# aharley/pips

Measured on AMD Instinct MI355X. Metric: particle-updates/sec (B*S*N*iters/s) at S=8 N=256 368x496, higher is better.
Workload: dtype f32; 1 GPU; BASELINE configs[1]: B=1/GPU S=8 368x496 N=256 I=6 fp32 stride 8, encoder included, inputs resident in HBM; clips_per_gpu=1, parallelism=clip-sharded x1, collective=none

## Files before the change

### include/pips_hip.h

```cpp
#ifndef PIPS_HIP_H
#define PIPS_HIP_H

#include <stddef.h>
#include <stdint.h>

#ifdef __cplusplus
extern "C" {
#endif

#define PIPS_OK            0
#define PIPS_E_ARG        -1
#define PIPS_E_WORKSPACE  -2
#define PIPS_E_LAUNCH     -3

#define PIPS_S        8
#define PIPS_C        128
#define PIPS_LEVELS   4
#define PIPS_RADIUS   3
#define PIPS_NCORR    196
#define PIPS_KIN      519
#define PIPS_KIN_PAD  544
#define PIPS_DMIX     512
#define PIPS_DEPTH    12
#define PIPS_NOUT     1040
// ... 128 lines not shown
                     float* C, int ldc, int M, int N, int K, int epi,
                     const float* R, int ldr, void* stream);
int    pips_conv_nhwc_f32(const float* in, int F, int H, int W, int Cin,
                          const float* wgt, const float* bias, int Cout, int ksize, int cstride, int pad,
                          float* out, float* stats, int* tiles_m_host, void* stream);

#define PIPS_EPI_BIAS      0
#define PIPS_EPI_GELU      1
#define PIPS_EPI_RESIDUAL  2
#define PIPS_EPI_RES_BF16  0x1000
int    pips_gemm_bf16(const void* A, int a_bf16, int lda, const void* W, const float* bias, void* C, int out_bf16, int ldc,
                      int M, int N, int K, int epi, const float* R, int ldr, void* stream);
int    pips_gemm_bf16_route(int M, int N, int K, int epi, int a_bf16, int out_bf16);

int    pips_gemm_f32_route(int M, int N, int K, int epi);
int    pips_device_cus(void);

int    pips_conv_nhwc_bf16(const float* in, int F, int H, int W, int Cin,
                           const void* wgt_bf16, const float* bias, int Cout, int ksize, int cstride, int pad,
                           float* out, float* stats, int* tiles_m_host, void* stream);

int    pips_conv_nhwc_bf16_maps(const void* in_bf16, const float* in_norm, int F, int H, int W, int Cin,
                                const void* wgt_bf16, const float* bias, int Cout, int ksize, int cstride, int pad,
                                void* out, int out_is_bf16, float* stats, int stats_parts_cap, int* tiles_m_host,
                                void* stream);

int    pips_split_bf16x3(const float* src, size_t n, void* dst3, void* stream);
int    pips_gemm_f32x3(const float* A, int lda, const void* W3, const float* bias,
                       float* C, int ldc, int M, int N, int K, int epi,
                       const float* R, int ldr, void* stream);
// ... 26 lines not shown
```

### pips_amd/_lib.py

```python
from __future__ import annotations

import ctypes as C
import os
import threading

HERE = os.path.dirname(os.path.abspath(__file__))
LIB_PATH = os.path.join(HERE, "libpips_hip.so")

c_void_p, c_int, c_size_t, c_float = C.c_void_p, C.c_int, C.c_size_t, C.c_float
fp = c_void_p

SIGNATURES = {
    "pips_last_error": (C.c_char_p, []),
    "pips_abi_version": (c_int, []),
    "pips_weight_arena_bytes": (c_size_t, []),
    "pips_repack_weights": (c_int, [C.POINTER(c_void_p), c_int, c_void_p, c_void_p]),
    "pips_repack_weights_ex": (c_int, [C.POINTER(c_void_p), c_int, c_void_p, c_int, c_void_p]),
    "pips_workspace_bytes": (c_size_t, [c_int] * 6),
    "pips_forward": (c_int, [c_void_p, fp, fp, fp, fp, fp, c_int, c_int, c_int, c_int, c_int, c_int, c_int, c_int,
                             c_void_p, c_size_t, fp, fp, fp, c_void_p]),
    "pips_forward_ce": (c_int, [c_void_p, fp, fp, fp, fp, fp, c_int, c_int, c_int, c_int, c_int, c_int, c_int, c_int,
                                c_void_p, c_size_t, fp, fp, fp, fp, fp, c_void_p, c_size_t, c_void_p]),
    "pips_track_ce": (c_int, [c_void_p, fp, c_int, c_int, c_int, c_int, fp, fp, fp, c_void_p, fp, c_int, c_int, c_int,
                              c_int, c_void_p, c_size_t, fp, fp, fp, fp, fp, c_void_p, c_size_t, c_void_p]),
# ... 45 lines not shown
    "pips_mixer_fwd": (c_int, [c_void_p, fp, c_int, fp, c_void_p, c_size_t, c_void_p]),
    "pips_mixer_fwd_bf16": (c_int, [c_void_p, fp, c_int, fp, c_void_p, c_size_t, c_void_p]),
    "pips_mixer_fwd_x3": (c_int, [c_void_p, fp, c_int, fp, c_void_p, c_size_t, c_void_p]),
    "pips_mixer_fwd_timed": (c_int, [c_void_p, fp, c_int, fp, c_void_p, c_size_t, c_void_p, C.POINTER(c_float)]),
    "pips_mixer_fwd_timed_ex": (c_int, [c_void_p, fp, c_int, c_int, fp, c_void_p, c_size_t, c_void_p,
                                        C.POINTER(c_float)]),
    "pips_mixer_gemm_train": (c_int, [c_void_p, c_int, c_int, c_void_p, c_size_t, c_void_p, c_int, C.POINTER(c_float)]),
    "pips_state_update": (c_int, [c_void_p, fp, fp, fp, fp, c_int, c_int, c_float, fp, fp, c_void_p]),
    "pips_gemm_f32": (c_int, [fp, c_int, fp, fp, fp, c_int, c_int, c_int, c_int, c_int, fp, c_int, c_void_p]),
    "pips_conv_nhwc_f32": (c_int, [fp, c_int, c_int, c_int, c_int, fp, fp, c_int, c_int, c_int, c_int, fp, fp,
                                   C.POINTER(c_int), c_void_p]),
    "pips_gemm_bf16": (c_int, [c_void_p, c_int, c_int, c_void_p, fp, c_void_p, c_int, c_int, c_int, c_int, c_int, c_int, fp, c_int,
                       c_void_p]),
    "pips_gemm_bf16_route": (c_int, [c_int] * 6),
    "pips_gemm_f32_route": (c_int, [c_int] * 4),
    "pips_device_cus": (c_int, []),
    "pips_conv_nhwc_bf16": (c_int, [fp, c_int, c_int, c_int, c_int, c_void_p, fp, c_int, c_int, c_int, c_int, fp, fp,
                                    C.POINTER(c_int), c_void_p]),
    "pips_conv_nhwc_bf16_maps": (c_int, [c_void_p, fp, c_int, c_int, c_int, c_int, c_void_p, fp, c_int, c_int, c_int, c_int,
                                         c_void_p, c_int, fp, c_int, C.POINTER(c_int), c_void_p]),
    "pips_split_bf16x3": (c_int, [fp, c_size_t, c_void_p, c_void_p]),
    "pips_gemm_f32x3": (c_int, [fp, c_int, c_void_p, fp, fp, c_int, c_int, c_int, c_int, c_int, fp, c_int, c_void_p]),
    "pips_conv_nhwc_f32x3": (c_int, [fp, c_int, c_int, c_int, c_int, c_void_p, fp, c_int, c_int, c_int, c_int, fp, fp,
                                     C.POINTER(c_int), c_void_p]),
}

_lock = threading.Lock()
_lib = None


# ... 45 lines not shown
```

### pips_amd/csrc/api.hip

```cpp
#include "common.h"

#include <cstdarg>
#include <cstdio>
#include <cstdlib>
#include <cstring>
#include <mutex>

namespace pips {

static thread_local char g_err[512] = "";

void set_error(const char* fmt, ...) {
    va_list ap;
    va_start(ap, fmt);
    vsnprintf(g_err, sizeof(g_err), fmt, ap);
    va_end(ap);
}

#ifdef PIPS_TUNING
int tune_env(const char* name, int dflt) {
    const char* e = getenv(name);
    return e ? atoi(e) : dflt;
}
#endif
// ... 774 lines not shown
    return gemm_h(reinterpret_cast<const float*>(A), a_bf16, lda, reinterpret_cast<const unsigned short*>(W), bias,
                  reinterpret_cast<float*>(C), out_bf16, ldc, M, N, K, epi, R, ldr, (hipStream_t)stream);
}

int pips_gemm_bf16_route(int M, int N, int K, int epi, int a_bf16, int out_bf16) {
    if (M <= 0 || N <= 0 || K <= 0) return 0;
    static const float dummy = 0.f;
    GemmArgs g;
    memset(&g, 0, sizeof(g));
    g.bias = &dummy; g.R = &dummy;
    g.M = M; g.N = N; g.K = K; g.lda = K; g.ldc = N; g.ldr = N; g.epi = epi;
    return gemm_bf16_asm_route(g, a_bf16, out_bf16);
}

int pips_device_cus(void) { return device_cus(); }

int pips_gemm_f32_route(int M, int N, int K, int epi) {
    if (M <= 0 || N <= 0 || K <= 0) return 0;
    static const float dummy = 0.f;
    GemmArgs g;
    memset(&g, 0, sizeof(g));
    g.bias = &dummy; g.R = &dummy;
    g.M = M; g.N = N; g.K = K; g.lda = K; g.ldc = N; g.ldr = N; g.epi = epi;
    return gemm_f32_t4_route(g, nullptr);
}

static int mixer_mode(int flags) {
    if (flags & PIPS_FLAG_SPLIT_BF16) return 2;
    if (flags & PIPS_FLAG_BF16_MIXER) return (flags & PIPS_FLAG_BF16_STREAM) ? 3 : 1;
    return 0;
// ... 441 lines not shown
```

### pips_amd/csrc/common.h

```cpp
#pragma once
#include <hip/hip_runtime.h>
#include <atomic>
#include <stdint.h>
#include <stddef.h>
#include "../../include/pips_hip.h"

namespace pips {

void set_error(const char* fmt, ...);

#define PIPS_CHECK_ARG(cond, ...)                                   \
    do {                                                            \
        if (!(cond)) { ::pips::set_error(__VA_ARGS__); return PIPS_E_ARG; } \
    } while (0)

#define PIPS_CHECK_LAUNCH(what)                                                     \
    do {                                                                            \
        hipError_t e__ = hipGetLastError();                                         \
        if (e__ != hipSuccess) {                                                    \
            ::pips::set_error("%s: %s", what, hipGetErrorString(e__));              \
            return PIPS_E_LAUNCH;                                                   \
        }                                                                           \
    } while (0)

// ... 197 lines not shown
                    typedef __bf16 bf16x4_ __attribute__((ext_vector_type(4)));
                    const f32x4_ t = {lo.x, lo.y, hi.x, hi.y};
                    bf16x4_ ob = __builtin_convertvector(t, bf16x4_);
                    *reinterpret_cast<uint2*>(reinterpret_cast<unsigned short*>(Cv) + o) = *reinterpret_cast<uint2*>(&ob);
                } else {
                    *reinterpret_cast<float4*>(reinterpret_cast<float*>(Cv) + o) = make_float4(lo.x, lo.y, hi.x, hi.y);
                }
            }
    }
}

int launch_gemm(const GemmArgs& a, hipStream_t st);
int gemm_f32_t4_route(const GemmArgs& a, int* tpb);
int launch_gemm_f32_t4(const GemmArgs& a, int route, int tpb, hipStream_t st);
int launch_conv(const GemmArgs& a, int frames, int* tiles_m, hipStream_t st);
int conv_f32_t4_config(const GemmArgs& a, int frames);
int launch_conv_f32_t4(const GemmArgs& a, int cfg, int frames, int* parts_out, hipStream_t st);
int launch_gemm_bf16(const GemmArgs& a, int a_bf16, int out_bf16, hipStream_t st);
int launch_conv_bf16(const GemmArgs& a, int frames, int* tiles_m, hipStream_t st, int in_bf16 = 0, int out_bf16 = 0);
int launch_conv3x3_c64_bf16(const GemmArgs& a, int frames, int* tiles_m, hipStream_t st, int in_bf16 = 0, int out_bf16 = 0);
bool conv3x3_c64_takes(int H, int W, int frames);
bool conv_c96_t4_takes(const GemmArgs& a, int frames, int in_bf16, int out_bf16);
int launch_conv_c96_t4(const GemmArgs& a, int frames, int* parts_out, hipStream_t st);
int gemm_bf16_asm_route(const GemmArgs& a, int a_bf16, int out_bf16);
bool gemm_bf16_t4_takes(const GemmArgs& a, int a_bf16, int out_bf16);
int launch_gemm_bf16_t4(const GemmArgs& a, hipStream_t st);
bool gemm_bf16_t4up_takes(const GemmArgs& a, int a_bf16, int out_bf16, int* tpb);
int launch_gemm_bf16_t4up(const GemmArgs& a, int tpb, hipStream_t st);
int launch_split_bf16x3(const float* src, size_t n, void* dst, hipStream_t st);
int launch_gemm_x3(const GemmArgs& a, hipStream_t st);
// ... 74 lines not shown
```

### pips_amd/csrc/gemm.hip

```cpp
#include "common.h"

#include <cstdlib>

namespace pips {



template <int BM, int BN, int WGM, int WGN, int KS, bool CONV>
__global__ __launch_bounds__(WGM * WGN * KS * 64, (BM * BN >= 128 * 128 && WGM * WGN * KS == 4) ? 2 : 1) void igemm_f32_kernel(GemmArgs p) {
    constexpr int NT = WGM * WGN * KS * 64;
    constexpr int BKB = 32 * KS;
    constexpr int LD = BKB + 4;
    constexpr int TPR = BKB / 4;
    constexpr int WTM = BM / WGM, WTN = BN / WGN;
    constexpr int TM = WTM / 32, TN = WTN / 32;
    constexpr int ROWS_PER_PASS = NT / TPR;
    constexpr int PA = BM / ROWS_PER_PASS, PB = BN / ROWS_PER_PASS;
    constexpr int STAGE = (BM + BN) * LD;
    static_assert(BM % ROWS_PER_PASS == 0 && BN % ROWS_PER_PASS == 0, "tile/loader mismatch");
    static_assert(WTM % 32 == 0 && WTN % 32 == 0, "wave tile must be 32-granular");
    static_assert(KS == 1 || (KS - 1) * BM * BN <= 2 * STAGE, "K-split reduction does not fit the stages");

    extern __shared__ __attribute__((aligned(16))) float smem[];

    const int tid = threadIdx.x;
    const int lane = tid & 63, wave = tid >> 6;
    const int ks = wave / (WGM * WGN);
    const int wmn = wave - ks * (WGM * WGN);
    const int wm = wmn / WGN, wn = wmn % WGN;
    const int l31 = lane & 31, half = lane >> 5;
    const Tile3 tile_ = xcd_tile_order(p.swz != 0);
    const int bx = tile_.x, by = tile_.y;
    const int m0 = bx * BM, n0 = by * BN;
    const int frame = tile_.z;
#ifdef PIPS_GEMM_TRACE
    unsigned long long* tr_ = p.trace + 8 * (size_t)(blockIdx.x + gridDim.x * (blockIdx.y + gridDim.y * blockIdx.z));
// ... 9 lines not shown
#define PIPS_T(slot)
#endif
    PIPS_T(0)

    const float* __restrict__ Abase = p.A;
    float* __restrict__ Cbase = p.C;
    if (CONV) {
        Abase += (size_t)frame * p.H * p.Win * p.Cin;
        Cbase += (size_t)frame * p.M * p.ldc;
    }

    const int lrow = tid / TPR, cg = tid % TPR;
    static_assert(PA <= 4 && PB <= 6, "extend the pass macros");
#define PIPS_PASSES_A(X) X(0) X(1) X(2) X(3)
#define PIPS_PASSES_B(X) X(0) X(1) X(2) X(3) X(4) X(5)
#define PIPS_DECL_A(i) int a_hi##i = 0, a_wi##i = 0; unsigned a_off##i = 0; float4 ra##i = make_float4(0.f, 0.f, 0.f, 0.f);
#define PIPS_DECL_B(i) unsigned b_off##i = 0; float4 rb##i = make_float4(0.f, 0.f, 0.f, 0.f);
    PIPS_PASSES_A(PIPS_DECL_A)
    PIPS_PASSES_B(PIPS_DECL_B)
#define PIPS_INIT_A(i)                                                        \
    if constexpr (i < PA) {                                                   \
        int m_ = m0 + lrow + i * ROWS_PER_PASS;                               \
        m_ = m_ < p.M ? m_ : p.M - 1;                                         \
        if (CONV) {                                                           \
            const int ho_ = m_ / p.Wo, wo_ = m_ - ho_ * p.Wo;                 \
            a_hi##i = ho_ * p.cstride - p.pad;                                \
            a_wi##i = wo_ * p.cstride - p.pad;                                \
        } else {                                                              \
            a_off##i = (unsigned)m_ * (unsigned)p.lda + cg * 4;               \
        }                                                                     \
    }
#define PIPS_INIT_B(i)                                                        \
// ... 9 lines not shown
    f32x16 acc[TM][TN];
#pragma unroll
    for (int i = 0; i < TM; ++i)
#pragma unroll
        for (int j = 0; j < TN; ++j)
#pragma unroll
            for (int r = 0; r < 16; ++r) acc[i][j][r] = 0.f;

#define PIPS_LOADC_A(i)                                                                             \
    if constexpr (i < PA) {                                                                         \
        const int hi_ = a_hi##i + kh_, wi_ = a_wi##i + kw_;                                         \
        const bool ok_ = (unsigned)hi_ < (unsigned)p.H && (unsigned)wi_ < (unsigned)p.Win;          \
        const int hc_ = ok_ ? hi_ : 0, wc_ = ok_ ? wi_ : 0;                                         \
        const float4 v_ = *reinterpret_cast<const float4*>(                                         \
            Abase + ((size_t)hc_ * p.Win + wc_) * p.Cin + c0_ + cg * 4);                            \
        ra##i = ok_ ? v_ : make_float4(0.f, 0.f, 0.f, 0.f);                                         \
    }
#define PIPS_LOADP_A(i) \
    if constexpr (i < PA) ra##i = *reinterpret_cast<const float4*>(Abase + a_off##i + k0_);
#define PIPS_LOAD_B(i) \
    if constexpr (i < PB) rb##i = *reinterpret_cast<const float4*>(p.W + b_off##i + k0_);
#define PIPS_LOAD_TILES(kb_)                                                                        \
    {                                                                                               \
        const int k0_ = (kb_) * BKB;                                                                \
        if (CONV) {                                                                                 \
                                 \
            const int tap_ = k0_ / p.Cin;                                                           \
            const int c0_ = k0_ - tap_ * p.Cin;                                                     \
            const int kh_ = tap_ / p.KW, kw_ = tap_ - kh_ * p.KW;                                   \
            PIPS_PASSES_A(PIPS_LOADC_A)                                                             \
        } else {                                                                                    \
            PIPS_PASSES_A(PIPS_LOADP_A)                                                             \
        }                                                                                           \
        PIPS_PASSES_B(PIPS_LOAD_B)                                                                  \
    }
#define PIPS_STORE_A(i) \
    if constexpr (i < PA) *reinterpret_cast<float4*>(&As_[(lrow + i * ROWS_PER_PASS) * LD + cg * 4]) = ra##i;
#define PIPS_STORE_B(i) \
    if constexpr (i < PB) *reinterpret_cast<float4*>(&Bs_[(lrow + i * ROWS_PER_PASS) * LD + cg * 4]) = rb##i;
#define PIPS_STORE_TILES(buf_)                                                                      \
    {                                                                                               \
        float* As_ = smem + (buf_) * STAGE;                                                         \
        float* Bs_ = As_ + BM * LD;                                                                 \
        PIPS_PASSES_A(PIPS_STORE_A)                                                                 \
        PIPS_PASSES_B(PIPS_STORE_B)                                                                 \
    }
#define PIPS_FRAGS(dst_a, dst_b, kk_)                                                               \
    {                                                                                               \
        _Pragma("unroll") for (int i = 0; i < TM; ++i)                                              \
            dst_a[i] = *reinterpret_cast<const float4*>(a_frag + i * 32 * LD + (kk_) * 8);          \
        _Pragma("unroll") for (int j = 0; j < TN; ++j)                                              \
            dst_b[j] = *reinterpret_cast<const float4*>(b_frag + j * 32 * LD + (kk_) * 8);          \
    }
#define PIPS_MFMA1(c_)                                                                              \
        _Pragma("unroll") for (int i = 0; i < TM; ++i)                                              \
            _Pragma("unroll") for (int j = 0; j < TN; ++j)                                          \
                acc[i][j] = CONV ? __builtin_amdgcn_mfma_f32_32x32x2f32(fa_[i].c_, fb_[j].c_, acc[i][j], 0, 0, 0) \
                                 : __builtin_amdgcn_mfma_f32_32x32x2f32(fb_[j].c_, fa_[i].c_, acc[i][j], 0, 0, 0);
#define PIPS_MFMA4(fa, fb)                                                                          \
    {                                                                                               \
        const float4* fa_ = fa; const float4* fb_ = fb;                                             \
// ... 3 lines not shown
    {                                                                                               \
        const float* a_frag = smem + (buf_) * STAGE + (wm * WTM + l31) * LD + ks * 32 + half * 4;   \
        const float* b_frag = smem + (buf_) * STAGE + BM * LD + (wn * WTN + l31) * LD + ks * 32 + half * 4; \
        float4 fa0[TM], fb0[TN], fa1[TM], fb1[TN];                                                  \
        PIPS_FRAGS(fa0, fb0, 0);                                                                    \
        PIPS_FRAGS(fa1, fb1, 1);                                                                    \
        PIPS_MFMA4(fa0, fb0);                                                                       \
        PIPS_FRAGS(fa0, fb0, 2);                                                                    \
        PIPS_MFMA4(fa1, fb1);                                                                       \
        PIPS_FRAGS(fa1, fb1, 3);                                                                    \
        PIPS_MFMA4(fa0, fb0);                                                                       \
        PIPS_MFMA4(fa1, fb1);                                                                       \
    }

    const int nk = p.K / BKB;
    PIPS_LOAD_TILES(0);
    PIPS_STORE_TILES(0);
    __syncthreads();
    PIPS_T(1)
#ifdef PIPS_GEMM_TRACE
    const long long cyc0_ = clock64();
#endif
    int buf = 0;
#ifdef PIPS_GEMM_ABLATE
    const bool ab_ld = !(p.epi & 0x100), ab_st = !(p.epi & 0x200), ab_bar = !(p.epi & 0x400);
    for (int kb = 0; kb + 1 < nk; ++kb) {
        if (ab_ld) PIPS_LOAD_TILES(kb + 1);
        asm volatile("" ::: "memory");
        PIPS_COMPUTE(buf);
        asm volatile("" ::: "memory");
        if (ab_st) PIPS_STORE_TILES(buf ^ 1);
        if (ab_bar) __syncthreads();
        buf ^= 1;
    }
#else
    for (int kb = 0; kb + 1 < nk; ++kb) {
        PIPS_LOAD_TILES(kb + 1);
        asm volatile("" ::: "memory");
        PIPS_COMPUTE(buf);
        asm volatile("" ::: "memory");
        PIPS_STORE_TILES(buf ^ 1);
        __syncthreads();
        buf ^= 1;
    }
#endif
    PIPS_COMPUTE(buf);
    PIPS_T(2)
#ifdef PIPS_GEMM_TRACE
    if (tid == 0) tr_[7] = (unsigned long long)(clock64() - cyc0_);
#endif
#undef PIPS_LOAD_TILES
#undef PIPS_STORE_TILES
#undef PIPS_PASSES_A
#undef PIPS_PASSES_B
#undef PIPS_DECL_A
#undef PIPS_DECL_B
#undef PIPS_INIT_A
#undef PIPS_INIT_B
#undef PIPS_LOADC_A
#undef PIPS_LOADP_A
#undef PIPS_LOAD_B
#undef PIPS_STORE_A
#undef PIPS_STORE_B
#undef PIPS_FRAGS
#undef PIPS_MFMA1
#undef PIPS_MFMA4
#undef PIPS_COMPUTE

    if (KS > 1) {
        __syncthreads();
        float* red = smem;
        if (ks > 0) {
#pragma unroll
            for (int i = 0; i < TM; ++i)
#pragma unroll
                for (int j = 0; j < TN; ++j)
#pragma unroll
                    for (int r = 0; r < 16; ++r)
                        red[((((ks - 1) * (WGM * WGN) + wmn) * (TM * TN) + i * TN + j) * 16 + r) * 64 + lane] =
                            acc[i][j][r];
        }
        __syncthreads();
// ... 119 lines not shown
    static void* buf = nullptr;
    if (!buf) { (void)hipMalloc(&buf, 8u << 20); (void)hipMemset(buf, 0, 8u << 20); }
    return reinterpret_cast<unsigned long long*>(buf);
}
extern "C" int pips_trace_read(void* host, size_t bytes) {
    return (int)hipMemcpy(host, trace_buffer(), bytes, hipMemcpyDeviceToHost);
}
#endif

static int swizzle_on(bool conv, long tiles, const GemmArgs& a) {
    const int force = PIPS_TUNE("PIPS_GEMM_SWZ", -1);
    if (force >= 0) return force != 0 && tiles >= 64;
    return !conv && (long long)a.M * (a.N > a.K ? a.N : a.K) * 4 > (256ll << 20);
}

template <int BM, int BN, int WGM, int WGN, int KS, bool CONV>
static int launch_tile(const GemmArgs& a_in, int frames, hipStream_t st) {
    static_assert(!CONV || KS == 1, "conv statistics assume KS == 1");
    GemmArgs a = a_in;
    dim3 grid(cdiv(a.M, BM), cdiv(a.N, BN), frames);
    dim3 block(WGM * WGN * KS * 64);
    a.swz = swizzle_on(CONV, (long)grid.x * grid.y * grid.z, a);
    size_t lds = (size_t)2 * (BM + BN) * (32 * KS + 4) * sizeof(float);
    auto kern = igemm_f32_kernel<BM, BN, WGM, WGN, KS, CONV>;
    if (lds > 64 * 1024) {
        static std::atomic<unsigned long long> raised{0};
        const int rc = ensure_dynamic_lds(raised, (const void*)kern, lds);
        if (rc != PIPS_OK) return rc;
    }
#ifdef PIPS_GEMM_TRACE
    a.trace = trace_buffer();
#endif
    hipLaunchKernelGGL(kern, grid, block, lds, st, a);
    PIPS_CHECK_LAUNCH("igemm_f32_kernel");
    return PIPS_OK;
}

static int forced_tile(const GemmArgs& a) {
    const int all = PIPS_TUNE("PIPS_GEMM_TILE", -1), up = PIPS_TUNE("PIPS_GEMM_TILE_UP", -1),
// ... 37 lines not shown
    if (b128 >= 400) return launch_tile<128, 128, 2, 2, 1, false>(a, 1, st);
    if (b64 >= 800 || !k64) return launch_tile<64, 64, 2, 2, 1, false>(a, 1, st);
    return launch_tile<64, 64, 2, 2, 2, false>(a, 1, st);
}

static void conv_tile(int rows, int cout, int frames, int* bm, int* bn) {
    int n = (cout % 128 == 0) ? 128 : (cout % 96 == 0 ? 96 : 64);
    long blocks128 = (long)cdiv(rows, 128) * (cout / n) * frames;
    *bm = (blocks128 >= 384 && n != 64) ? 128 : 64;
    if (*bm == 64 && n == 128 && (long)cdiv(rows, 64) * (cout / 128) * frames < 400) n = 64;
    *bn = n;
    const int force_bm = PIPS_TUNE("PIPS_CONV_BM", 0);
    if (force_bm == 64 || force_bm == 128) *bm = force_bm;
}

int launch_conv(const GemmArgs& a, int frames, int* tiles_m, hipStream_t st) {
    PIPS_CHECK_ARG(a.Cin % 32 == 0, "conv: Cin=%d must be a multiple of 32", a.Cin);
    PIPS_CHECK_ARG(a.N % 32 == 0 && (a.N % 64 == 0 || a.N % 96 == 0), "conv: unsupported Cout=%d", a.N);
    PIPS_CHECK_ARG(a.K == a.KH * a.KW * a.Cin, "conv: K mismatch");
    {
        const int cfg = conv_f32_t4_config(a, frames);
        if (cfg >= 0) return launch_conv_f32_t4(a, cfg, frames, tiles_m, st);
    }
    int bm, bn;
    conv_tile(a.M, a.N, frames, &bm, &bn);
    if (tiles_m) *tiles_m = cdiv(a.M, bm) * ((bn == 96 && bm == 128) ? 4 : 2);
    if (bn == 128) {
        return bm == 128 ? launch_tile<128, 128, 2, 2, 1, true>(a, frames, st)
                         : launch_tile<64, 128, 2, 2, 1, true>(a, frames, st);
    } else if (bn == 96) {
        return bm == 128 ? launch_tile<128, 96, 4, 1, 1, true>(a, frames, st)
                         : launch_tile<64, 96, 2, 1, 1, true>(a, frames, st);
    }
    return bm == 128 ? launch_tile<128, 64, 2, 2, 1, true>(a, frames, st)
                     : launch_tile<64, 64, 2, 2, 1, true>(a, frames, st);
}

}
```

### pips_amd/csrc/gemm_bf16.hip

```cpp
#include "common.h"

#include <cstdlib>

namespace pips {

typedef float f32x8 __attribute__((ext_vector_type(8)));
typedef __bf16 bf16x8 __attribute__((ext_vector_type(8)));
typedef __bf16 bf16x4 __attribute__((ext_vector_type(4)));

__device__ __forceinline__ uint4 pack_bf16x8(const float4& lo, const float4& hi) {
    f32x8 v = {lo.x, lo.y, lo.z, lo.w, hi.x, hi.y, hi.z, hi.w};
    bf16x8 b = __builtin_convertvector(v, bf16x8);
    return *reinterpret_cast<uint4*>(&b);
}

template <int BM, int BN, int WGM, int WGN, int KS, bool A_BF16, bool OUT_BF16, int BKE = 64, bool CONV = false>
__global__ __launch_bounds__(WGM * WGN * KS * 64, (BM * BN >= 128 * 128 && WGM * WGN * KS == 4) ? 2 : 1) void gemm_bf16_kernel(GemmArgs p) {
    constexpr int NT = WGM * WGN * KS * 64;
    constexpr int BKB = BKE * KS;
    static_assert(!CONV || KS == 1, "conv: no K split");
    constexpr int LDB = BKB * 2 + 16;
    constexpr int TPR = BKB / 8;
    constexpr int WTM = BM / WGM, WTN = BN / WGN;
    constexpr int TM = WTM / 32, TN = WTN / 32;
// ... 78 lines not shown
        } else {                                                                                     \
            ra##i##l = *reinterpret_cast<const float4*>(Af + a_off##i + k0_);                        \
            ra##i##h = *reinterpret_cast<const float4*>(Af + a_off##i + k0_ + 4);                    \
        }                                                                                            \
    }                                                                                                \
    if constexpr (i < PB) rb##i = *reinterpret_cast<const uint4*>(Wb + b_off##i + k0_);
#define PIPS_LOAD_TILES(kb_)                                                                         \
    {                                                                                                \
        const int k0_ = (kb_) * BKB;                                                                 \
        const int tap_ = CONV ? k0_ / p.Cin : 0;             \
        const int c0_ = CONV ? k0_ - tap_ * p.Cin : 0;                                               \
        const int kh_ = CONV ? tap_ / p.KW : 0, kw_ = CONV ? tap_ - kh_ * p.KW : 0;                  \
        (void)c0_; (void)kh_; (void)kw_;                                                             \
        PIPS_PASSES(PIPS_LOAD)                                                                       \
    }
#define PIPS_STORE(i)                                                                                \
    if constexpr (i < PA)                                                                            \
        *reinterpret_cast<uint4*>(As_ + (lrow + i * ROWS_PER_PASS) * LDB + cg * 16) =               \
            A_BF16 ? rq##i : pack_bf16x8(ra##i##l, ra##i##h);                                        \
    if constexpr (i < PB)                                                                            \
        *reinterpret_cast<uint4*>(Bs_ + (lrow + i * ROWS_PER_PASS) * LDB + cg * 16) = rb##i;
#define PIPS_STORE_TILES(buf_) { char* As_ = smem + (buf_) * STAGE; char* Bs_ = As_ + BM * LDB; PIPS_PASSES(PIPS_STORE) }
#define PIPS_COMPUTE(buf_)                                                                           \
    {                                                                                                \
        const char* a_frag = smem + (buf_) * STAGE + (wm * WTM + l31) * LDB + ks * (BKE * 2) + half * 16;  \
        const char* b_frag = smem + (buf_) * STAGE + BM * LDB + (wn * WTN + l31) * LDB + ks * (BKE * 2) + half * 16; \
        _Pragma("unroll") for (int kk = 0; kk < BKE / 16; ++kk) {                                    \
            uint4 fa[TM], fb[TN];                                                                    \
            _Pragma("unroll") for (int i = 0; i < TM; ++i)                                           \
                fa[i] = *reinterpret_cast<const uint4*>(a_frag + i * 32 * LDB + kk * 32);            \
            _Pragma("unroll") for (int j = 0; j < TN; ++j)                                           \
                fb[j] = *reinterpret_cast<const uint4*>(b_frag + j * 32 * LDB + kk * 32);            \
            _Pragma("unroll") for (int i = 0; i < TM; ++i)                                           \
                _Pragma("unroll") for (int j = 0; j < TN; ++j)                                       \
                    acc[i][j] = CONV ? __builtin_amdgcn_mfma_f32_32x32x16_bf16(                      \
                                           *reinterpret_cast<const bf16x8*>(&fa[i]),                 \
                                           *reinterpret_cast<const bf16x8*>(&fb[j]), acc[i][j], 0, 0, 0) \
                                     : __builtin_amdgcn_mfma_f32_32x32x16_bf16(                      \
                                           *reinterpret_cast<const bf16x8*>(&fb[j]),                 \
                                           *reinterpret_cast<const bf16x8*>(&fa[i]), acc[i][j], 0, 0, 0); \
        }                                                                                            \
    }

    const int nk = p.K / BKB;
    PIPS_LOAD_TILES(0);
    PIPS_STORE_TILES(0);
    __syncthreads();
    int buf = 0;
    for (int kb = 0; kb + 1 < nk; ++kb) {
        PIPS_LOAD_TILES(kb + 1);
        asm volatile("" ::: "memory");
        PIPS_COMPUTE(buf);
        asm volatile("" ::: "memory");
        PIPS_STORE_TILES(buf ^ 1);
        __syncthreads();
        buf ^= 1;
    }
    PIPS_COMPUTE(buf);
#undef PIPS_PASSES
#undef PIPS_DECL
#undef PIPS_INIT
#undef PIPS_LOAD
#undef PIPS_LOAD_TILES
#undef PIPS_STORE
#undef PIPS_STORE_TILES
#undef PIPS_COMPUTE

    if (KS > 1) {
        __syncthreads();
        float* red = reinterpret_cast<float*>(smem);
        if (ks > 0) {
#pragma unroll
            for (int i = 0; i < TM; ++i)
#pragma unroll
                for (int j = 0; j < TN; ++j)
#pragma unroll
                    for (int r = 0; r < 16; ++r)
                        red[((((ks - 1) * (WGM * WGN) + wmn) * (TM * TN) + i * TN + j) * 16 + r) * 64 + lane] =
                            acc[i][j][r];
        }
// ... 242 lines not shown
```

### pips_amd/csrc/gemm_x3.hip

```cpp
#include "gemm_tail.h"

#include <cstdlib>

#ifndef PIPS_X3_ABL
#define PIPS_X3_ABL 0
#endif

namespace pips {

typedef __bf16 bf16x8 __attribute__((ext_vector_type(8)));

__device__ __forceinline__ unsigned cvt_pk_bf16(float a, float b) {
    typedef float f32x2_ __attribute__((ext_vector_type(2)));
    typedef __bf16 bf16x2_ __attribute__((ext_vector_type(2)));
    const f32x2_ v = {a, b};
    const bf16x2_ r = __builtin_convertvector(v, bf16x2_);
    return *reinterpret_cast<const unsigned*>(&r);
}
__device__ __forceinline__ void split3_pair(float x0, float x1, unsigned& h, unsigned& m, unsigned& l) {
    h = cvt_pk_bf16(x0, x1);
    const float r0 = x0 - __uint_as_float(h << 16), r1 = x1 - __uint_as_float(h & 0xffff0000u);
    m = cvt_pk_bf16(r0, r1);
    const float s0 = r0 - __uint_as_float(m << 16), s1 = r1 - __uint_as_float(m & 0xffff0000u);
    l = cvt_pk_bf16(s0, s1);
// ... 118 lines not shown
            na##i##h = *reinterpret_cast<const float4*>(Af + a_off##i + k0_ + 4);                    \
        }                                                                                            \
    }
#define PIPS_LOAD_B(i, pl)                                                                           \
    if constexpr (i < PB) nb##i##pl = *reinterpret_cast<const uint4*>(Wb + pl * wplane + b_off##i + k0_);
#define PIPS_LOAD(i) PIPS_LOAD_A(i) PIPS_LOAD_B(i, 0) PIPS_LOAD_B(i, 1) PIPS_LOAD_B(i, 2)
#define PIPS_ROTATE(i)                                                                               \
    ra##i##l = na##i##l; ra##i##h = na##i##h; rb##i##0 = nb##i##0; rb##i##1 = nb##i##1; rb##i##2 = nb##i##2;
#define PIPS_KCOORDS(kb_)                                                                            \
        const int k0_ = (PIPS_X3_ABL & 16) ? 0 : (kb_) * BKB;     \
        const int tap_ = CONV ? k0_ / p.Cin : 0;              \
        const int c0_ = CONV ? k0_ - tap_ * p.Cin : 0;                                               \
        const int kh_ = CONV ? tap_ / p.KW : 0, kw_ = CONV ? tap_ - kh_ * p.KW : 0;                  \
        (void)c0_; (void)kh_; (void)kw_;
#define PIPS_LOAD_TILES(kb_) { PIPS_KCOORDS(kb_) PIPS_PASSES(PIPS_LOAD) }
#define PIPS_STORE(i)                                                                                \
    if constexpr (i < PA) {                                                                          \
        uint4 h_, m_, l_;                                                                            \
        if (PIPS_X3_ABL & 1) { h_ = *reinterpret_cast<uint4*>(&ra##i##l); m_ = *reinterpret_cast<uint4*>(&ra##i##h); l_ = h_; } \
        else split3_x8(ra##i##l, ra##i##h, h_, m_, l_);                                              \
        char* dst_ = As_ + (lrow + i * RPP) * LDB + wchunk;                                         \
        *reinterpret_cast<uint4*>(dst_) = h_;                                                        \
        *reinterpret_cast<uint4*>(dst_ + PLANE_A) = m_;                                              \
        *reinterpret_cast<uint4*>(dst_ + 2 * PLANE_A) = l_;                                          \
    }                                                                                                \
    if constexpr (i < PB) {                                                                          \
        char* dst_ = Bs_ + (lrow + i * RPP) * LDB + wchunk;                                         \
        *reinterpret_cast<uint4*>(dst_) = rb##i##0;                                                  \
        *reinterpret_cast<uint4*>(dst_ + PLANE_B) = rb##i##1;                                        \
        *reinterpret_cast<uint4*>(dst_ + 2 * PLANE_B) = rb##i##2;                                    \
    }
#define PIPS_STORE_TILES(buf_) { char* As_ = smem + (buf_) * STAGE; char* Bs_ = As_ + 3 * PLANE_A; PIPS_PASSES(PIPS_STORE) }
#define PIPS_MFMA(fa, fb, pa_, pb_)                                                                  \
    _Pragma("unroll") for (int i = 0; i < TM; ++i)                                                   \
        _Pragma("unroll") for (int j = 0; j < TN; ++j)                                               \
            acc[i][j] = CONV ? __builtin_amdgcn_mfma_f32_32x32x16_bf16(                              \
                                   *reinterpret_cast<const bf16x8*>(&fa[pa_][i]),                    \
                                   *reinterpret_cast<const bf16x8*>(&fb[pb_][j]), acc[i][j], 0, 0, 0) \
                             : __builtin_amdgcn_mfma_f32_32x32x16_bf16(                              \
                                   *reinterpret_cast<const bf16x8*>(&fb[pb_][j]),                    \
                                   *reinterpret_cast<const bf16x8*>(&fa[pa_][i]), acc[i][j], 0, 0, 0);
#define PIPS_FRAGS(fa, fb, buf_, kk_)                                                                \
    {                                                                                                \
        const char* a_frag = smem + (buf_) * STAGE + (wm * WTM + l31) * LDB + ((kk_) ? rchunk1 : rchunk0);     \
        const char* b_frag = smem + (buf_) * STAGE + 3 * PLANE_A + (wn * WTN + l31) * LDB + ((kk_) ? rchunk1 : rchunk0); \
        _Pragma("unroll") for (int pl = 0; pl < 3; ++pl) {                                           \
            _Pragma("unroll") for (int i = 0; i < TM; ++i)                                           \
                fa[pl][i] = *reinterpret_cast<const uint4*>(a_frag + pl * PLANE_A + i * 32 * LDB);   \
            _Pragma("unroll") for (int j = 0; j < TN; ++j)                                           \
                fb[pl][j] = *reinterpret_cast<const uint4*>(b_frag + pl * PLANE_B + j * 32 * LDB);   \
        }                                                                                            \
    }
#define PIPS_MFMA3A(fa, fb) PIPS_MFMA(fa, fb, 2, 0) PIPS_MFMA(fa, fb, 0, 2) PIPS_MFMA(fa, fb, 1, 1)
#define PIPS_MFMA3B(fa, fb) PIPS_MFMA(fa, fb, 1, 0) PIPS_MFMA(fa, fb, 0, 1) PIPS_MFMA(fa, fb, 0, 0)
#define PIPS_SB __builtin_amdgcn_sched_barrier(0);

    const int nk = p.K / BKB;
    if constexpr (BKE == 16) {
        uint4 fa0[3][TM], fb0[3][TN];
        PIPS_LOAD_TILES(0);
        PIPS_PASSES(PIPS_ROTATE)
        PIPS_STORE_TILES(0);
        PIPS_LOAD_TILES(nk > 1 ? 1 : 0);
        __syncthreads();
        int buf = 0;
        for (int kb = 0; kb + 1 < nk; ++kb) {
            PIPS_PASSES(PIPS_ROTATE)
            PIPS_KCOORDS(kb + 2 < nk ? kb + 2 : nk - 1)
            PIPS_FRAGS(fa0, fb0, buf, 0);
            PIPS_SB
            PIPS_MFMA(fa0, fb0, 2, 0) PIPS_LOAD_A(0) PIPS_LOAD_B(0, 0) PIPS_SB
            PIPS_MFMA(fa0, fb0, 0, 2) PIPS_LOAD_A(1) PIPS_LOAD_B(0, 1) PIPS_SB
            PIPS_MFMA(fa0, fb0, 1, 1) PIPS_LOAD_B(0, 2) PIPS_LOAD_B(1, 0) PIPS_SB
            PIPS_MFMA(fa0, fb0, 1, 0) PIPS_LOAD_B(1, 1) PIPS_LOAD_B(1, 2) PIPS_SB
            PIPS_MFMA(fa0, fb0, 0, 1) PIPS_MFMA(fa0, fb0, 0, 0)
            PIPS_STORE_TILES(buf ^ 1);
            __syncthreads();
            buf ^= 1;
        }
        PIPS_FRAGS(fa0, fb0, buf, 0);
        PIPS_MFMA3A(fa0, fb0) PIPS_MFMA3B(fa0, fb0)
    } else {
    uint4 fa0[3][TM], fb0[3][TN], fa1[3][TM], fb1[3][TN];
    PIPS_LOAD_TILES(0);
    PIPS_PASSES(PIPS_ROTATE)
    PIPS_STORE_TILES(0);
    PIPS_LOAD_TILES(nk > 1 ? 1 : 0);
    __syncthreads();
    int buf = 0;
    PIPS_FRAGS(fa0, fb0, 0, 0);
    for (int kb = 0; kb + 1 < nk; ++kb) {
        PIPS_PASSES(PIPS_ROTATE)
        PIPS_KCOORDS(kb + 2 < nk ? kb + 2 : nk - 1)
        PIPS_SB
        PIPS_FRAGS(fa1, fb1, buf, 1);
        PIPS_SB
        PIPS_MFMA(fa0, fb0, 2, 0) if (!(PIPS_X3_ABL & 2)) { PIPS_LOAD_A(0) } PIPS_SB
        PIPS_MFMA(fa0, fb0, 0, 2) if (!(PIPS_X3_ABL & 2)) { PIPS_LOAD_A(1) PIPS_LOAD_B(0, 0) } PIPS_SB
        PIPS_MFMA(fa0, fb0, 1, 1) if (!(PIPS_X3_ABL & 2)) { PIPS_LOAD_B(0, 1) PIPS_LOAD_B(0, 2) } PIPS_SB
        PIPS_MFMA(fa0, fb0, 1, 0) if (!(PIPS_X3_ABL & 2)) { PIPS_LOAD_B(1, 0) PIPS_LOAD_B(1, 1) } PIPS_SB
        PIPS_MFMA(fa0, fb0, 0, 1) if (!(PIPS_X3_ABL & 2)) { PIPS_LOAD_B(1, 2) } PIPS_SB
        PIPS_MFMA(fa0, fb0, 0, 0)
        PIPS_MFMA3A(fa1, fb1)
        if (!(PIPS_X3_ABL & 4)) PIPS_STORE_TILES(buf ^ 1);
        if (!(PIPS_X3_ABL & 8)) __syncthreads();
        PIPS_FRAGS(fa0, fb0, buf ^ 1, 0);
        PIPS_SB
        PIPS_MFMA3B(fa1, fb1)
        buf ^= 1;
    }
    PIPS_FRAGS(fa1, fb1, buf, 1);
    PIPS_MFMA3A(fa0, fb0) PIPS_MFMA3B(fa0, fb0)
    PIPS_MFMA3A(fa1, fb1) PIPS_MFMA3B(fa1, fb1)
    }
#undef PIPS_PASSES
#undef PIPS_DECL
#undef PIPS_INIT
#undef PIPS_LOAD
#undef PIPS_LOAD_A
#undef PIPS_LOAD_B
#undef PIPS_KCOORDS
#undef PIPS_ROTATE
#undef PIPS_LOAD_TILES
#undef PIPS_STORE
#undef PIPS_STORE_TILES
#undef PIPS_MFMA
#undef PIPS_FRAGS
#undef PIPS_MFMA3A
#undef PIPS_MFMA3B
#undef PIPS_SB

    __builtin_amdgcn_sched_barrier(0);
    asm volatile("s_nop 11");
    __builtin_amdgcn_sched_barrier(0);

    if (!ksplit_reduce<KS, WGM * WGN, TM, TN>(acc, reinterpret_cast<float*>(smem), ks, wmn, lane)) return;

    if (CONV) {
        conv_epilogue<BM, BN, WGM, WTM, WTN, NT, TM, TN>(acc, p, p.C + (size_t)frame * p.M * p.ldc,
                                                        reinterpret_cast<float*>(smem), frame, tile_.x, m0, n0,
// ... 84 lines not shown
```

Measured before the change: 1.389 million particle-updates/s.

## Add two-deep global prefetch variant for f32 implicit-GEMM conv tiles

Adds a PF=2 template variant of the f32 implicit-GEMM kernel that keeps two K blocks of global loads in flight in two register sets, swapping them each step, and defers the conv padding mask to the LDS store. It is routed for 64x64 and 128x96 conv tiles when the grid is small (at most 1024 tiles), and is meant to hide global load latency on under-occupied encoder convs. The cost is a doubled register footprint for the staging loads, which may lower occupancy or cause spills. Also adds a route query API and a tuning sweep, and renames the store macros.

```diff
diff --git a/include/pips_hip.h b/include/pips_hip.h
--- a/include/pips_hip.h
+++ b/include/pips_hip.h
@@ -166,6 +166,7 @@
 int    pips_gemm_bf16_route(int M, int N, int K, int epi, int a_bf16, int out_bf16);
 
 int    pips_gemm_f32_route(int M, int N, int K, int epi);
+int    pips_conv_f32_route(int F, int H, int W, int Cin, int Cout, int ksize, int cstride, int pad);
 int    pips_device_cus(void);
 
 int    pips_conv_nhwc_bf16(const float* in, int F, int H, int W, int Cin,
diff --git a/pips_amd/_lib.py b/pips_amd/_lib.py
--- a/pips_amd/_lib.py
+++ b/pips_amd/_lib.py
@@ -83,6 +83,7 @@
                        c_void_p]),
     "pips_gemm_bf16_route": (c_int, [c_int] * 6),
     "pips_gemm_f32_route": (c_int, [c_int] * 4),
+    "pips_conv_f32_route": (c_int, [c_int] * 8),
     "pips_device_cus": (c_int, []),
     "pips_conv_nhwc_bf16": (c_int, [fp, c_int, c_int, c_int, c_int, c_void_p, fp, c_int, c_int, c_int, c_int, fp, fp,
                                     C.POINTER(c_int), c_void_p]),
diff --git a/pips_amd/csrc/api.hip b/pips_amd/csrc/api.hip
--- a/pips_amd/csrc/api.hip
+++ b/pips_amd/csrc/api.hip
@@ -812,6 +812,19 @@
 }
 
 int pips_device_cus(void) { return device_cus(); }
+
+int pips_conv_f32_route(int F, int H, int W, int Cin, int Cout, int ksize, int cstride, int pad) {
+    if (F <= 0 || H <= 0 || W <= 0 || Cin <= 0 || Cout <= 0) return 0;
+    GemmArgs g;
+    memset(&g, 0, sizeof(g));
+    g.H = H; g.Win = W; g.Cin = Cin; g.KH = g.KW = ksize; g.cstride = cstride; g.pad = pad;
+    g.Ho = conv_out(H, ksize, cstride, pad); g.Wo = conv_out(W, ksize, cstride, pad);
+    if (g.Ho <= 0 || g.Wo <= 0) return 0;
+    g.M = g.Ho * g.Wo; g.N = Cout; g.K = ksize * ksize * Cin; g.ldc = Cout; g.epi = EPI_BIAS;
+    static float dummy = 0.f;
+    g.bias = &dummy; g.stats = &dummy;
+    return conv_f32_route(g, F);
+}
 
 int pips_gemm_f32_route(int M, int N, int K, int epi) {
     if (M <= 0 || N <= 0 || K <= 0) return 0;
diff --git a/pips_amd/csrc/common.h b/pips_amd/csrc/common.h
--- a/pips_amd/csrc/common.h
+++ b/pips_amd/csrc/common.h
@@ -235,6 +235,7 @@
 int gemm_f32_t4_route(const GemmArgs& a, int* tpb);
 int launch_gemm_f32_t4(const GemmArgs& a, int route, int tpb, hipStream_t st);
 int launch_conv(const GemmArgs& a, int frames, int* tiles_m, hipStream_t st);
+int conv_f32_route(const GemmArgs& a, int frames);
 int conv_f32_t4_config(const GemmArgs& a, int frames);
 int launch_conv_f32_t4(const GemmArgs& a, int cfg, int frames, int* parts_out, hipStream_t st);
 int launch_gemm_bf16(const GemmArgs& a, int a_bf16, int out_bf16, hipStream_t st);
diff --git a/pips_amd/csrc/gemm.hip b/pips_amd/csrc/gemm.hip
--- a/pips_amd/csrc/gemm.hip
+++ b/pips_amd/csrc/gemm.hip
@@ -6,7 +6,7 @@
 
 
 
-template <int BM, int BN, int WGM, int WGN, int KS, bool CONV>
+template <int BM, int BN, int WGM, int WGN, int KS, bool CONV, int PF = 1>
 __global__ __launch_bounds__(WGM * WGN * KS * 64, (BM * BN >= 128 * 128 && WGM * WGN * KS == 4) ? 2 : 1) void igemm_f32_kernel(GemmArgs p) {
     constexpr int NT = WGM * WGN * KS * 64;
     constexpr int BKB = 32 * KS;
@@ -20,6 +20,7 @@
     static_assert(BM % ROWS_PER_PASS == 0 && BN % ROWS_PER_PASS == 0, "tile/loader mismatch");
     static_assert(WTM % 32 == 0 && WTN % 32 == 0, "wave tile must be 32-granular");
     static_assert(KS == 1 || (KS - 1) * BM * BN <= 2 * STAGE, "K-split reduction does not fit the stages");
+    static_assert(PF == 1 || PF == 2, "one or two K blocks in flight");
 
     extern __shared__ __attribute__((aligned(16))) float smem[];
 
@@ -59,8 +60,9 @@
     static_assert(PA <= 4 && PB <= 6, "extend the pass macros");
 #define PIPS_PASSES_A(X) X(0) X(1) X(2) X(3)
 #define PIPS_PASSES_B(X) X(0) X(1) X(2) X(3) X(4) X(5)
-#define PIPS_DECL_A(i) int a_hi##i = 0, a_wi##i = 0; unsigned a_off##i = 0; float4 ra##i = make_float4(0.f, 0.f, 0.f, 0.f);
-#define PIPS_DECL_B(i) unsigned b_off##i = 0; float4 rb##i = make_float4(0.f, 0.f, 0.f, 0.f);
+#define PIPS_DECL_A(i) int a_hi##i = 0, a_wi##i = 0; unsigned a_off##i = 0; float4 ra##i = make_float4(0.f, 0.f, 0.f, 0.f); \
+    float4 qa##i = make_float4(0.f, 0.f, 0.f, 0.f); bool ka##i = true, kq##i = true;
+#define PIPS_DECL_B(i) unsigned b_off##i = 0; float4 rb##i = make_float4(0.f, 0.f, 0.f, 0.f); float4 qb##i = make_float4(0.f, 0.f, 0.f, 0.f);
     PIPS_PASSES_A(PIPS_DECL_A)
     PIPS_PASSES_B(PIPS_DECL_B)
 #define PIPS_INIT_A(i)                                                        \
@@ -100,7 +102,10 @@
         const int hc_ = ok_ ? hi_ : 0, wc_ = ok_ ? wi_ : 0;                                         \
         const float4 v_ = *reinterpret_cast<const float4*>(                                         \
             Abase + ((size_t)hc_ * p.Win + wc_) * p.Cin + c0_ + cg * 4);                            \
-        ra##i = ok_ ? v_ : make_float4(0.f, 0.f, 0.f, 0.f);                                         \
+         \
+             \
+        if constexpr (PF == 2) { ra##i = v_; ka##i = ok_; }                                          \
+        else ra##i = ok_ ? v_ : make_float4(0.f, 0.f, 0.f, 0.f);                                    \
     }
 #define PIPS_LOADP_A(i) \
     if constexpr (i < PA) ra##i = *reinterpret_cast<const float4*>(Abase + a_off##i + k0_);
@@ -120,17 +125,29 @@
         }                                                                                           \
         PIPS_PASSES_B(PIPS_LOAD_B)                                                                  \
     }
-#define PIPS_STORE_A(i) \
-    if constexpr (i < PA) *reinterpret_cast<float4*>(&As_[(lrow + i * ROWS_PER_PASS) * LD + cg * 4]) = ra##i;
-#define PIPS_STORE_B(i) \
+#define PIPS_LDS_PUT_A(i)                                                                           \
+    if constexpr (i < PA) {                                                                         \
+        if constexpr (PF == 2 && CONV) {                                                            \
+            float x_ = ra##i.x, y_ = ra##i.y, z_ = ra##i.z, w_ = ra##i.w;                           \
+            asm volatile("" : "+v"(x_), "+v"(y_), "+v"(z_), "+v"(w_));                              \
+            ra##i = make_float4(x_, y_, z_, w_);                                                    \
+        }                                                                                           \
+        *reinterpret_cast<float4*>(&As_[(lrow + i * ROWS_PER_PASS) * LD + cg * 4]) =                \
+            (PF == 2 && CONV && !ka##i) ? make_float4(0.f, 0.f, 0.f, 0.f) : ra##i;                  \
+    }
+#define PIPS_LDS_PUT_B(i) \
     if constexpr (i < PB) *reinterpret_cast<float4*>(&Bs_[(lrow + i * ROWS_PER_PASS) * LD + cg * 4]) = rb##i;
-#define PIPS_STORE_TILES(buf_)                                                                      \
+#define PIPS_LDS_PUT_TILES(buf_)                                                                      \
     {                                                                                               \
         float* As_ = smem + (buf_) * STAGE;                                                         \
         float* Bs_ = As_ + BM * LD;                                                                 \
-        PIPS_PASSES_A(PIPS_STORE_A)                                                                 \
-        PIPS_PASSES_B(PIPS_STORE_B)                                                                 \
-    }
+        PIPS_PASSES_A(PIPS_LDS_PUT_A)                                                                 \
+        PIPS_PASSES_B(PIPS_LDS_PUT_B)                                                                 \
+    }
+#define PIPS_SWAP_A(i) \
+    if constexpr (i < PA) { const float4 t_ = ra##i; ra##i = qa##i; qa##i = t_; const bool k_ = ka##i; ka##i = kq##i; kq##i = k_; }
+#define PIPS_SWAP_B(i) \
+    if constexpr (i < PB) { const float4 t_ = rb##i; rb##i = qb##i; qb##i = t_; }
 #define PIPS_FRAGS(dst_a, dst_b, kk_)                                                               \
     {                                                                                               \
         _Pragma("unroll") for (int i = 0; i < TM; ++i)                                              \
@@ -164,14 +181,59 @@
     }
 
     const int nk = p.K / BKB;
+    int buf = 0;
+#ifdef PIPS_GEMM_TRACE
+    long long cyc0_ = 0;
+#endif
+    if constexpr (PF == 2) {
+#define PIPS_SWAP_SETS                                                                              \
+        {                                                                                           \
+            PIPS_PASSES_A(PIPS_SWAP_A)                                                              \
+            PIPS_PASSES_B(PIPS_SWAP_B)                                                              \
+        }
+        PIPS_LOAD_TILES(0);
+        PIPS_LDS_PUT_TILES(0);
+        PIPS_LOAD_TILES(nk > 1 ? 1 : 0);
+        PIPS_SWAP_SETS
+        PIPS_LOAD_TILES(nk > 2 ? 2 : nk - 1);
+        __syncthreads();
+        PIPS_T(1)
+#ifdef PIPS_GEMM_TRACE
+        cyc0_ = clock64();
+#endif
+        int kb = 0;
+        for (; kb + 2 < nk; kb += 2) {
+            asm volatile("" ::: "memory");
+            PIPS_COMPUTE(0);
+            asm volatile("" ::: "memory");
+            PIPS_SWAP_SETS
+            PIPS_LDS_PUT_TILES(1);
+            __syncthreads();
+            PIPS_LOAD_TILES(kb + 3 < nk ? kb + 3 : nk - 1);
+            asm volatile("" ::: "memory");
+            PIPS_COMPUTE(1);
+            asm volatile("" ::: "memory");
+            PIPS_SWAP_SETS
+            PIPS_LDS_PUT_TILES(0);
+            __syncthreads();
+            PIPS_LOAD_TILES(kb + 4 < nk ? kb + 4 : nk - 1);
+        }
+        if (kb + 1 < nk) {
+            PIPS_COMPUTE(0);
+            asm volatile("" ::: "memory");
+            PIPS_SWAP_SETS
+            PIPS_LDS_PUT_TILES(1);
+            __syncthreads();
+            buf = 1;
+        }
+    } else {
     PIPS_LOAD_TILES(0);
-    PIPS_STORE_TILES(0);
+    PIPS_LDS_PUT_TILES(0);
     __syncthreads();
     PIPS_T(1)
 #ifdef PIPS_GEMM_TRACE
-    const long long cyc0_ = clock64();
-#endif
-    int buf = 0;
+    cyc0_ = clock64();
+#endif
 #ifdef PIPS_GEMM_ABLATE
     const bool ab_ld = !(p.epi & 0x100), ab_st = !(p.epi & 0x200), ab_bar = !(p.epi & 0x400);
     for (int kb = 0; kb + 1 < nk; ++kb) {
@@ -179,7 +241,7 @@
         asm volatile("" ::: "memory");
         PIPS_COMPUTE(buf);
         asm volatile("" ::: "memory");
-        if (ab_st) PIPS_STORE_TILES(buf ^ 1);
+        if (ab_st) PIPS_LDS_PUT_TILES(buf ^ 1);
         if (ab_bar) __syncthreads();
         buf ^= 1;
     }
@@ -189,18 +251,19 @@
         asm volatile("" ::: "memory");
         PIPS_COMPUTE(buf);
         asm volatile("" ::: "memory");
-        PIPS_STORE_TILES(buf ^ 1);
+        PIPS_LDS_PUT_TILES(buf ^ 1);
         __syncthreads();
         buf ^= 1;
     }
 #endif
+    }
     PIPS_COMPUTE(buf);
     PIPS_T(2)
 #ifdef PIPS_GEMM_TRACE
     if (tid == 0) tr_[7] = (unsigned long long)(clock64() - cyc0_);
 #endif
 #undef PIPS_LOAD_TILES
-#undef PIPS_STORE_TILES
+#undef PIPS_LDS_PUT_TILES
 #undef PIPS_PASSES_A
 #undef PIPS_PASSES_B
 #undef PIPS_DECL_A
@@ -210,12 +273,15 @@
 #undef PIPS_LOADC_A
 #undef PIPS_LOADP_A
 #undef PIPS_LOAD_B
-#undef PIPS_STORE_A
-#undef PIPS_STORE_B
+#undef PIPS_LDS_PUT_A
+#undef PIPS_LDS_PUT_B
 #undef PIPS_FRAGS
 #undef PIPS_MFMA1
 #undef PIPS_MFMA4
 #undef PIPS_COMPUTE
+#undef PIPS_SWAP_SETS
+#undef PIPS_SWAP_A
+#undef PIPS_SWAP_B
 
     if (KS > 1) {
         __syncthreads();
@@ -365,7 +431,7 @@
     return !conv && (long long)a.M * (a.N > a.K ? a.N : a.K) * 4 > (256ll << 20);
 }
 
-template <int BM, int BN, int WGM, int WGN, int KS, bool CONV>
+template <int BM, int BN, int WGM, int WGN, int KS, bool CONV, int PF = 1>
 static int launch_tile(const GemmArgs& a_in, int frames, hipStream_t st) {
     static_assert(!CONV || KS == 1, "conv statistics assume KS == 1");
     GemmArgs a = a_in;
@@ -373,7 +439,7 @@
     dim3 block(WGM * WGN * KS * 64);
     a.swz = swizzle_on(CONV, (long)grid.x * grid.y * grid.z, a);
     size_t lds = (size_t)2 * (BM + BN) * (32 * KS + 4) * sizeof(float);
-    auto kern = igemm_f32_kernel<BM, BN, WGM, WGN, KS, CONV>;
+    auto kern = igemm_f32_kernel<BM, BN, WGM, WGN, KS, CONV, PF>;
     if (lds > 64 * 1024) {
         static std::atomic<unsigned long long> raised{0};
         const int rc = ensure_dynamic_lds(raised, (const void*)kern, lds);
@@ -441,10 +507,70 @@
     if (force_bm == 64 || force_bm == 128) *bm = force_bm;
 }
 
+#ifdef PIPS_TUNING
+static int sweep_tile(const GemmArgs& a, int frames, int* tiles_m, hipStream_t st) {
+    const int id = tune_env("PIPS_CONV_TILE", -1);
+    int bm = 0, wgm = 0;
+    switch (id) {
+        case 0: bm = 64; wgm = 2; break;
+        case 1: bm = 64; wgm = 2; break;
+        case 2: bm = 128; wgm = 4; break;
+        case 3: bm = 128; wgm = 4; break;
+        case 4: bm = 64; wgm = 2; break;
+        case 5: bm = 32; wgm = 1; break;
+        case 6: bm = 128; wgm = 4; break;
+        case 7: bm = 64; wgm = 2; break;
+        case 8: bm = 32; wgm = 1; break;
+        case 9: bm = 64; wgm = 2; break;
+        case 10: bm = 64; wgm = 2; break;
+        case 11: bm = 128; wgm = 4; break;
+        case 12: bm = 32; wgm = 1; break;
+        case 13: bm = 64; wgm = 2; break;
+        case 14: bm = 64; wgm = 2; break;
+        case 15: bm = 64; wgm = 2; break;
+        default: return -1;
+    }
+    if (tiles_m) *tiles_m = cdiv(a.M, bm) * wgm;
+    switch (id) {
+        case 0: return launch_tile<64, 64, 2, 2, 1, true>(a, frames, st);
+        case 1: return launch_tile<64, 128, 2, 2, 1, true>(a, frames, st);
+        case 2: return launch_tile<128, 128, 4, 2, 1, true>(a, frames, st);
+        case 3: return launch_tile<128, 64, 4, 2, 1, true>(a, frames, st);
+        case 4: return launch_tile<64, 32, 2, 1, 1, true>(a, frames, st);
+        case 5: return launch_tile<32, 64, 1, 2, 1, true>(a, frames, st);
+        case 6: return launch_tile<128, 96, 4, 1, 1, true>(a, frames, st);
+        case 7: return launch_tile<64, 96, 2, 1, 1, true>(a, frames, st);
+        case 8: return launch_tile<32, 32, 1, 1, 1, true>(a, frames, st);
+        case 9: return launch_tile<64, 128, 2, 4, 1, true>(a, frames, st);
+        case 10: return launch_tile<64, 64, 2, 2, 1, true, 2>(a, frames, st);
+        case 11: return launch_tile<128, 96, 4, 1, 1, true, 2>(a, frames, st);
+        case 12: return launch_tile<32, 32, 1, 1, 1, true, 2>(a, frames, st);
+        case 13: return launch_tile<64, 128, 2, 4, 1, true, 2>(a, frames, st);
+        case 14: return launch_tile<64, 32, 2, 1, 1, true, 2>(a, frames, st);
+        default: return launch_tile<64, 96, 2, 1, 1, true, 2>(a, frames, st);
+    }
+}
+#endif
+
+bool conv_deep_prefetch(const GemmArgs& a, int frames, int bm, int bn) {
+    if (!((bm == 64 && bn == 64) || (bm == 128 && bn == 96))) return false;
+    return (long)cdiv(a.M, bm) * cdiv(a.N, bn) * frames <= 1024 && PIPS_TUNE("PIPS_CONV_PF2", 1);
+}
+
+int conv_f32_route(const GemmArgs& a, int frames) {
+    if (conv_f32_t4_config(a, frames) >= 0) return 1;
+    int bm, bn;
+    conv_tile(a.M, a.N, frames, &bm, &bn);
+    return conv_deep_prefetch(a, frames, bm, bn) ? 2 : 0;
+}
+
 int launch_conv(const GemmArgs& a, int frames, int* tiles_m, hipStream_t st) {
     PIPS_CHECK_ARG(a.Cin % 32 == 0, "conv: Cin=%d must be a multiple of 32", a.Cin);
     PIPS_CHECK_ARG(a.N % 32 == 0 && (a.N % 64 == 0 || a.N % 96 == 0), "conv: unsupported Cout=%d", a.N);
     PIPS_CHECK_ARG(a.K == a.KH * a.KW * a.Cin, "conv: K mismatch");
+#ifdef PIPS_TUNING
+    if (tune_env("PIPS_CONV_TILE", -1) >= 0) return sweep_tile(a, frames, tiles_m, st);
+#endif
     {
         const int cfg = conv_f32_t4_config(a, frames);
         if (cfg >= 0) return launch_conv_f32_t4(a, cfg, frames, tiles_m, st);
@@ -452,6 +578,10 @@
     int bm, bn;
     conv_tile(a.M, a.N, frames, &bm, &bn);
     if (tiles_m) *tiles_m = cdiv(a.M, bm) * ((bn == 96 && bm == 128) ? 4 : 2);
+    if (conv_deep_prefetch(a, frames, bm, bn)) {
+        if (bn == 96 && bm == 128) return launch_tile<128, 96, 4, 1, 1, true, 2>(a, frames, st);
+        if (bn == 64 && bm == 64) return launch_tile<64, 64, 2, 2, 1, true, 2>(a, frames, st);
+    }
     if (bn == 128) {
         return bm == 128 ? launch_tile<128, 128, 2, 2, 1, true>(a, frames, st)
                          : launch_tile<64, 128, 2, 2, 1, true>(a, frames, st);
diff --git a/pips_amd/csrc/gemm_bf16.hip b/pips_amd/csrc/gemm_bf16.hip
--- a/pips_amd/csrc/gemm_bf16.hip
+++ b/pips_amd/csrc/gemm_bf16.hip
@@ -116,13 +116,13 @@
         (void)c0_; (void)kh_; (void)kw_;                                                             \
         PIPS_PASSES(PIPS_LOAD)                                                                       \
     }
-#define PIPS_STORE(i)                                                                                \
+#define PIPS_LDS_PUT(i)                                                                                \
     if constexpr (i < PA)                                                                            \
         *reinterpret_cast<uint4*>(As_ + (lrow + i * ROWS_PER_PASS) * LDB + cg * 16) =               \
             A_BF16 ? rq##i : pack_bf16x8(ra##i##l, ra##i##h);                                        \
     if constexpr (i < PB)                                                                            \
         *reinterpret_cast<uint4*>(Bs_ + (lrow + i * ROWS_PER_PASS) * LDB + cg * 16) = rb##i;
-#define PIPS_STORE_TILES(buf_) { char* As_ = smem + (buf_) * STAGE; char* Bs_ = As_ + BM * LDB; PIPS_PASSES(PIPS_STORE) }
+#define PIPS_LDS_PUT_TILES(buf_) { char* As_ = smem + (buf_) * STAGE; char* Bs_ = As_ + BM * LDB; PIPS_PASSES(PIPS_LDS_PUT) }
 #define PIPS_COMPUTE(buf_)                                                                           \
     {                                                                                                \
         const char* a_frag = smem + (buf_) * STAGE + (wm * WTM + l31) * LDB + ks * (BKE * 2) + half * 16;  \
@@ -146,7 +146,7 @@
 
     const int nk = p.K / BKB;
     PIPS_LOAD_TILES(0);
-    PIPS_STORE_TILES(0);
+    PIPS_LDS_PUT_TILES(0);
     __syncthreads();
     int buf = 0;
     for (int kb = 0; kb + 1 < nk; ++kb) {
@@ -154,7 +154,7 @@
         asm volatile("" ::: "memory");
         PIPS_COMPUTE(buf);
         asm volatile("" ::: "memory");
-        PIPS_STORE_TILES(buf ^ 1);
+        PIPS_LDS_PUT_TILES(buf ^ 1);
         __syncthreads();
         buf ^= 1;
     }
@@ -164,8 +164,8 @@
 #undef PIPS_INIT
 #undef PIPS_LOAD
 #undef PIPS_LOAD_TILES
-#undef PIPS_STORE
-#undef PIPS_STORE_TILES
+#undef PIPS_LDS_PUT
+#undef PIPS_LDS_PUT_TILES
 #undef PIPS_COMPUTE
 
     if (KS > 1) {
diff --git a/pips_amd/csrc/gemm_x3.hip b/pips_amd/csrc/gemm_x3.hip
--- a/pips_amd/csrc/gemm_x3.hip
+++ b/pips_amd/csrc/gemm_x3.hip
@@ -156,7 +156,7 @@
         const int kh_ = CONV ? tap_ / p.KW : 0, kw_ = CONV ? tap_ - kh_ * p.KW : 0;                  \
         (void)c0_; (void)kh_; (void)kw_;
 #define PIPS_LOAD_TILES(kb_) { PIPS_KCOORDS(kb_) PIPS_PASSES(PIPS_LOAD) }
-#define PIPS_STORE(i)                                                                                \
+#define PIPS_LDS_PUT(i)                                                                                \
     if constexpr (i < PA) {                                                                          \
         uint4 h_, m_, l_;                                                                            \
         if (PIPS_X3_ABL & 1) { h_ = *reinterpret_cast<uint4*>(&ra##i##l); m_ = *reinterpret_cast<uint4*>(&ra##i##h); l_ = h_; } \
@@ -172,7 +172,7 @@
         *reinterpret_cast<uint4*>(dst_ + PLANE_B) = rb##i##1;                                        \
         *reinterpret_cast<uint4*>(dst_ + 2 * PLANE_B) = rb##i##2;                                    \
     }
-#define PIPS_STORE_TILES(buf_) { char* As_ = smem + (buf_) * STAGE; char* Bs_ = As_ + 3 * PLANE_A; PIPS_PASSES(PIPS_STORE) }
+#define PIPS_LDS_PUT_TILES(buf_) { char* As_ = smem + (buf_) * STAGE; char* Bs_ = As_ + 3 * PLANE_A; PIPS_PASSES(PIPS_LDS_PUT) }
 #define PIPS_MFMA(fa, fb, pa_, pb_)                                                                  \
     _Pragma("unroll") for (int i = 0; i < TM; ++i)                                                   \
         _Pragma("unroll") for (int j = 0; j < TN; ++j)                                               \
@@ -202,7 +202,7 @@
         uint4 fa0[3][TM], fb0[3][TN];
         PIPS_LOAD_TILES(0);
         PIPS_PASSES(PIPS_ROTATE)
-        PIPS_STORE_TILES(0);
+        PIPS_LDS_PUT_TILES(0);
         PIPS_LOAD_TILES(nk > 1 ? 1 : 0);
         __syncthreads();
         int buf = 0;
@@ -216,7 +216,7 @@
             PIPS_MFMA(fa0, fb0, 1, 1) PIPS_LOAD_B(0, 2) PIPS_LOAD_B(1, 0) PIPS_SB
             PIPS_MFMA(fa0, fb0, 1, 0) PIPS_LOAD_B(1, 1) PIPS_LOAD_B(1, 2) PIPS_SB
             PIPS_MFMA(fa0, fb0, 0, 1) PIPS_MFMA(fa0, fb0, 0, 0)
-            PIPS_STORE_TILES(buf ^ 1);
+            PIPS_LDS_PUT_TILES(buf ^ 1);
             __syncthreads();
             buf ^= 1;
         }
@@ -226,7 +226,7 @@
     uint4 fa0[3][TM], fb0[3][TN], fa1[3][TM], fb1[3][TN];
     PIPS_LOAD_TILES(0);
     PIPS_PASSES(PIPS_ROTATE)
-    PIPS_STORE_TILES(0);
+    PIPS_LDS_PUT_TILES(0);
     PIPS_LOAD_TILES(nk > 1 ? 1 : 0);
     __syncthreads();
     int buf = 0;
@@ -244,7 +244,7 @@
         PIPS_MFMA(fa0, fb0, 0, 1) if (!(PIPS_X3_ABL & 2)) { PIPS_LOAD_B(1, 2) } PIPS_SB
         PIPS_MFMA(fa0, fb0, 0, 0)
         PIPS_MFMA3A(fa1, fb1)
-        if (!(PIPS_X3_ABL & 4)) PIPS_STORE_TILES(buf ^ 1);
+        if (!(PIPS_X3_ABL & 4)) PIPS_LDS_PUT_TILES(buf ^ 1);
         if (!(PIPS_X3_ABL & 8)) __syncthreads();
         PIPS_FRAGS(fa0, fb0, buf ^ 1, 0);
         PIPS_SB
@@ -264,8 +264,8 @@
 #undef PIPS_KCOORDS
 #undef PIPS_ROTATE
 #undef PIPS_LOAD_TILES
-#undef PIPS_STORE
-#undef PIPS_STORE_TILES
+#undef PIPS_LDS_PUT
+#undef PIPS_LDS_PUT_TILES
 #undef PIPS_MFMA
 #undef PIPS_FRAGS
 #undef PIPS_MFMA3A
```

Result: faster. 1.405 million particle-updates/s (median of 6 runs) (+1.1%).
